# awslabs/palace

Hardware: AMD Instinct MI355X
Metric: curl-curl Mult DOF/s + PCG iters/s, p=3 H(curl) 10M DOF @1/2/4/8 GPU (higher is better)
Workload: dtype f64

## Files before the change

palace_amd/csrc/pa_internal.hpp:

```cpp
#pragma once

#include <hip/hip_runtime.h>

#include <cstdint>
#include <cstdio>
#include <memory>
#include <stdexcept>
#include <string>
#include <vector>

#include "../../include/palace_amd.h"
#include "pa_devbuf.hpp"
#include "pa_stream_host.hpp"

struct pa_op;
typedef struct pa_op pa_op_fwd;

struct pa_csr {
  bool symmetric = true;
  int32_t nrows = 0;
  int32_t ncols = 0;
  int64_t nnz = 0;
  pa::DevBuf<int32_t> d_rowptr, d_col;
  pa::DevBuf<double> d_val;
// ... 70 lines not shown
  DevBuf<double> d_geom;
  Ref<QData> metric;
  DevBuf<int32_t> d_attr_e;
  std::vector<int32_t> h_attr;
  std::vector<int32_t> eorder;
  std::vector<double> w1;
  DevBuf<double> d_xnodes, d_gtab;
  std::vector<double> wq;
  int refcount = 1;
  virtual ~Geom() = default;
};

struct CoeffDev {
  const int32_t *attr_mat = nullptr;
  const double *mat = nullptr;
  int nattr = 0;
};

struct CoeffHost {
  std::vector<int32_t> attr_mat;
  std::vector<double> mat;
  int dim = 3;
  size_t slots = 0;
  DevBuf<int32_t> d_attr_mat;
  DevBuf<double> d_mat;
  DevBuf<double> d_mat_t;
  bool symmetric() const { return !d_mat_t; }
  CoeffDev dev() const;
};

struct TransposeScope {
  TransposeScope(bool on);
  ~TransposeScope();
  static bool active();

private:
  bool prev_;
};

__host__ __device__ inline int nd_qd_cstride(int q1d) { return q1d == 5 ? 126 : q1d * q1d * q1d; }
__host__ __device__ inline int nd_qd_offset(int q1d, int c, int q) {
  if (q1d == 4) return ((c * 2 + (q >> 5)) * 16 + (q & 15)) * 2 + ((q >> 4) & 1);
  if (q1d == 5) {
    const int qz = q / 25, t = q - 25 * qz;
    return c * 126 + (qz < 4 ? (qz >> 1) * 50 + 2 * t + (qz & 1) : 100 + t);
  }
  return c * q1d * q1d * q1d + q;
}

enum StreamForm { kStreamPlain = 0, kStreamMasked = 1, kStreamAll = 2 };
inline StreamForm stream_form(bool masked) { return masked ? kStreamMasked : kStreamPlain; }

struct StreamTables {
  DevBuf<uint32_t> d_flags;
  DevBuf<uint32_t> d_rchunk;
  DevBuf<int32_t> d_rhdr;
  DevBuf<int32_t> d_rpos;
  int n_rows = 0, n_runs = 0;
  bool ready() const { return d_rhdr != nullptr; }
};

struct SubOp {
  Ref<Geom> geom;
  Ref<QData> qd;
  int fe_type = 0, p = 0, q1d = 0, P = 0, Q = 0, ne = 0, lsize = 0;
  int qf = 0;
  uint32_t trial_ops = 0, test_ops = 0;
  DevBuf<int32_t> d_lidx;
  DevBuf<int32_t> d_sidx;
  DevBuf<int32_t> d_sidx_bc;
  DevBuf<uint16_t> d_perm;
  DevBuf<uint16_t> d_perm_x;
  DevBuf<int32_t> d_shared;
  DevBuf<int32_t> d_shared_bc;
  std::vector<int32_t> h_shared;
  int n_shared = 0;
  std::vector<uint16_t> h_perm;
  std::vector<int32_t> h_sidx;
  DevBuf<double> d_ye;
  DevBuf<double> d_ye2;
  DevBuf<int32_t> d_tptr;
  DevBuf<int32_t> d_tent;
  DevBuf<uint32_t> d_idxc;
  bool stream_default = true;
  std::vector<uint32_t> h_perm_s;
  DevBuf<uint32_t> d_slots;
  int n_slot_patterns = 0;
  DevBuf<double> d_coef_s;
  std::vector<char> h_ess_flag;
  StreamTables stream[3];
  std::vector<double> Bc, Gc, Bo;
  DevBuf<double> d_tab;
  bool iso = false;
  std::vector<uint8_t> ctx_blob;
  CoeffHost c0, c1;
};

struct DenseSub {
  Ref<Geom> geom;
  int fe_type = 0, P = 0, Q = 0, Qpad = 0, nch = 0, ne = 0, nb = 0, lsize = 0, KP = 0, PT = 0;
  int qf = 0, mode = 0;
  bool contra = false;
  bool ye_rows = false;
  uint32_t trial_ops = 0, test_ops = 0;
  DevBuf<int32_t> d_idx;
  DevBuf<int32_t> d_idx_bc;
  DevBuf<uint8_t> d_ess_flag;
  DevBuf<uint16_t> d_co;
  DevBuf<uint32_t> d_co2;
  DevBuf<int32_t> d_rows;
  int n_rows = 0;
  std::vector<int32_t> h_idx;
  std::vector<int32_t> h_off;
  DevBuf<double> d_Tf, d_Tt;
  DevBuf<double> d_L;
  DevBuf<double> d_qdata;
  std::vector<uint16_t> h_co;
  double chk_interp = 0.0, chk_deriv = 0.0;
  DevBuf<double> d_ye2;
  DevBuf<uint8_t> d_affine;
  DevBuf<double> d_wrel;
  int n_affine = 0;
  DevBuf<int32_t> d_blist[2];
  int n_blist[2] = {0, 0};
  int L_rows = 0, ncq = 0, num_cu = 0;
  DevBuf<double> d_interp, d_deriv;
  DevBuf<int32_t> d_off;
  DevBuf<int8_t> d_cor;
  DevBuf<uint8_t> d_ori;
  DevBuf<double> d_ye;
  DevBuf<int32_t> d_tptr, d_tent;
  std::vector<uint8_t> ctx_blob;
  CoeffHost c0, c1;
};

struct MixedSide {
  int fe_type = 0, P = 0, lsize = 0, nc = 3;
  std::vector<int32_t> h_off;
  DevBuf<int32_t> d_sidx;
  DevBuf<int8_t> d_cor;
  DevBuf<double> d_tabF, d_tabT;
  DevBuf<int32_t> d_tptr, d_tent;
};
struct MixedSub {
  Ref<Geom> geom;
  int ne = 0, Q = 0, qf = 0, kind = 0;
  bool error = false;
  MixedSide s1, s2;
  CoeffHost c0, c1;
  DevBuf<double> d_ye;
  mutable DevBuf<double> d_ye_t;
  std::unique_ptr<SubOp> hex1, hex2;
  DevBuf<int32_t> d_eorder;
};

void parse_coeff(const void *blob, size_t bytes, int dim, CoeffHost &out, size_t slot_offset);

void launch_geom(const pa_mesh_desc &mesh, Geom &g, hipStream_t s);
void launch_nd_hex_apply(const SubOp &so, const double *x, double *y, double *ye, bool masked, hipStream_t s,
                         bool accumulate = true, int ess_policy = -1, const double *x1 = nullptr, double *y1 = nullptr,
                         double *ye1 = nullptr);
bool nd_hex_supports_two_rhs(const SubOp &so);
void launch_et_gather2(const SubOp &so, double *y0, double *y1, bool accumulate, hipStream_t s, const double *x0,
                       const double *x1, int ess_policy);
bool nd_hex_fuses_essential(const SubOp &so);
void finalize_exclusive(pa_op_fwd *op);
// ... 141 lines not shown
```

palace_amd/csrc/pa_nd_hex_stream.hip:

```cpp
#include <algorithm>
#include <map>

#include "pa_nd_hex_core.hpp"
#include "pa_stream_launch.hpp"

namespace pa {

typedef double d2v __attribute__((ext_vector_type(2)));

__host__ __device__ constexpr int stream_lds_elem(const int raw) { return (raw + 15) / 32 * 32 + 16; }

template <int P1>
struct NDStreamArgs {
  int ne, nbatch, chunk;
  const uint32_t *idxc;
  const uint32_t *flagw;
  const uint32_t *slots;
  const double *qdata;
  const double *qaff;
  const double *qcol;
  double wq2[2];
  double wqi2[2];
  const double *coef;
  const double *xn, *gtab;
  const double *x;
  double *y, *ye;
  const double *x1, *coef1;
  double *y1, *ye1;
  const double *qdata1;
  int qm[2], qc[2], qn[2];
  int nsplit;
  const double *xg0, *xg1;
  const unsigned long long *xg_sel;
  double *yg;
  NDTab<P1, 4> tab;
};

template <int P1, bool USE_U, bool USE_C, bool METRIC, int MINW, int GPOS, bool CPLX = false, bool SPLIT = false, int GEOMN = 0,
          bool COMPACT = false>
__global__ __launch_bounds__(64 * kWavesPerBlock, MINW) void nd_hex_stream_kernel(const NDStreamArgs<P1> a) {
  static_assert(!COMPACT || (!CPLX && !GEOMN), "the compact-only form: real kernels on packed or metric data");
  static_assert(!CPLX || (USE_U && USE_C), "the complex form is built on the curl-curl + mass kernels");
  static_assert(!(CPLX && SPLIT), "no split-vector form of the complex kernel");
  static_assert(!GEOMN || (!USE_U && USE_C && !METRIC && !CPLX), "geometry from the nodes: the curl-curl kernel");
  constexpr int Q1 = 4;
  constexpr bool AFF = (!CPLX || METRIC) && !GEOMN;
  constexpr bool EARLY_IDX = P1 < 3;
  using L = typename std::conditional<P1 == 3 && !CPLX && USE_C && !USE_U, NDLayoutInPlaceSwz3, NDLayout<P1, Q1>>::type;
  constexpr int NC = P1 + 1, PP = 3 * P1 * NC * NC, NPL = (PP + 15) / 16, NPK = (NPL + 3) / 4;
  constexpr int NG = METRIC ? (USE_U ? 7 : 6) : 6 * ((USE_U ? 1 : 0) + (USE_C ? 1 : 0));
  static_assert(PP <= 256, "8-bit slots");
  using streamhost::kIdxPattern;
  using streamhost::kIdxStart0;
  using streamhost::kIdxWords;
  constexpr int LDS_SIDE = (PP + 1) / 2 + (NPK + 1) * 8;
  constexpr int LDS_XN = GEOMN ? 82 : 0;
  constexpr int LDS_ELEM = stream_lds_elem(L::ELEM_PAD + LDS_SIDE + 12 + LDS_XN);
  extern __shared__ __attribute__((aligned(16))) double smem[];
  const int lane = threadIdx.x & 63;
  const int wave = __builtin_amdgcn_readfirstlane(threadIdx.x >> 6);
  const int xcd = blockIdx.x & 7;
  const int base = xcd * a.chunk, bend = min(base + a.chunk, a.nbatch);
  const int stride = (int)(gridDim.x >> 3) * kWavesPerBlock;
  int b = base + (int)(blockIdx.x >> 3) * kWavesPerBlock + wave;
  if (b >= bend) return;
  const double *xsel = (CPLX && ((lane >> 4) & 1)) ? a.x1 : a.x;
  const double *xgh = nullptr;
  if (SPLIT) xgh = ((a.xg_sel ? *a.xg_sel : 0ull) & 1ull) ? a.xg1 : a.xg0;
  auto load_idx = [&](const int bb, const int sub, const int t, int (&s)[NPL + 2], unsigned (&p)[NPK + 1]) {
    const int e = CPLX ? bb * 2 + (sub >> 1) : bb * 4 + sub;
    const uint32_t *ic = a.idxc + (size_t)e * kIdxWords;
#pragma unroll
    for (int r = 0; r < NPL; r++) s[r] = (int)__builtin_nontemporal_load(&ic[r]);
    s[NPL] = (int)__builtin_nontemporal_load(&ic[kIdxStart0 + t]);
    s[NPL + 1] = (int)__builtin_nontemporal_load(&ic[kIdxStart0 + 16 + (t & 3)]);
    p[NPK] = __builtin_nontemporal_load(&a.flagw[(size_t)e * 16 + t]);
    p[0] = __builtin_nontemporal_load(&ic[kIdxPattern]);
  };
  auto gather = [&](int (&s)[NPL + 2], unsigned (&p)[NPK + 1], double (&xv)[NPL], int *stab, const int t) {
    stab[t] = s[NPL];
    if (t < 4) stab[16 + t] = s[NPL + 1];
    wave_sync();
    const unsigned fw = p[NPK];
    {
      const uint32_t *sl = a.slots + (size_t)p[0] * (NPK * 16) + t;
#pragma unroll
      for (int k = 0; k < NPK; k++) p[k] = sl[16 * k];
    }
#pragma unroll
    for (int r = 0; r < NPL; r++) {
      const unsigned w = (unsigned)s[r], low = (w & 0xffffu) & ((2u << t) - 1u);
      const int rid = (int)((w >> 16) & 31u) + __popc(low) - 1;
      const int pos = low ? 16 * r + 31 - __clz((int)low) : (int)((w >> 21) & 255u);
      int dof = stab[rid] + (t + 16 * r - pos);
      if (!(16 * r + 15 < PP) && t + 16 * r >= PP) dof = 0;
      xv[r] = SPLIT ? (dof < a.nsplit ? xsel : xgh)[dof] : xsel[dof];
      const int word = dof | ((fw >> (2 * r + 1)) & 1u ? kExclBit : 0) | ((fw >> (18 + r)) & 1u ? kEssBit : 0);
      s[r] = (fw >> (2 * r)) & 1u ? -1 - word : word;
    }
  };
  auto settle = [&](unsigned (&p)[NPK + 1]) { asm volatile("" : "+v"(p[NPK])); };
  int sA[NPL + 2];
  unsigned pA[NPK + 1];
  double xv[NPL];
  load_idx(b, lane >> 4, lane & 15, sA, pA);
  gather(sA, pA, xv,
         reinterpret_cast<int *>(smem + (size_t)(wave * 4 + (lane >> 4)) * LDS_ELEM + L::ELEM_PAD + LDS_SIDE), lane & 15);
#pragma unroll
  for (int r = 0; r < NPL; r++) asm volatile("" : "+v"(xv[r]));
  settle(pA);

  d2v gq[(GEOMN || COMPACT) ? 1 : 2 * NG];
  double gr[COMPACT ? NG : 1];
  double xl[GEOMN ? 6 : 1];
  auto load_xn = [&](const int ee, const int t) {
    const double *xp = a.xn + (size_t)ee * 81;
#pragma unroll
    for (int r = 0; r < (GEOMN ? 6 : 1); r++) xl[r] = (t + 16 * r < 81) ? __builtin_nontemporal_load(&xp[t + 16 * r]) : 0.0;
  };
  auto load_q = [&](const int ee, const int t, const int kind) {
    if (GEOMN) return load_xn(ee, t);
    if (COMPACT) {
      constexpr int NS = METRIC ? 7 : NG;
      const int rs = kind == 2 ? 4 : 16;
      const double *g = kind == 2 ? a.qaff + ((size_t)ee * (4 * NS) + (t & 1)) : a.qcol + ((size_t)ee * (NS * 16) + t);
#pragma unroll
      for (int c = 0; c < NG; c++) gr[c] = __builtin_nontemporal_load(&g[rs * c]);
      return;
    }
    if (AFF && !(CPLX && !METRIC)) {
      constexpr int NS = METRIC ? 7 : NG;
      const int rs = kind == 2 ? 1 : (kind == 1 ? 4 : 16);
      const d2v *g = kind == 2   ? reinterpret_cast<const d2v *>(a.qaff) + (size_t)ee * (2 * NS)
                     : kind == 1 ? reinterpret_cast<const d2v *>(a.qcol) + ((size_t)ee * (NS * 8) + (t >> 1))
                                 : reinterpret_cast<const d2v *>(a.qdata) + ((size_t)ee * (2 * NS * 16) + t);
#pragma unroll
      for (int k = 0; k < 2 * NG; k++) gq[k] = __builtin_nontemporal_load(&g[rs * k]);
      return;
    }
    if (CPLX && !METRIC) {
      const int grp = (lane >> 4) & 1;
      const int mo = a.qm[grp], co = a.qc[grp];
      const d2v *g = reinterpret_cast<const d2v *>(grp ? a.qdata1 : a.qdata) + ((size_t)ee * (2 * a.qn[grp] * 16) + t);
      const d2v zero = {0.0, 0.0};
#pragma unroll
      for (int k = 0; k < 12; k++) {
        gq[k] = mo >= 0 ? __builtin_nontemporal_load(&g[16 * (2 * mo + k)]) : zero;
        gq[12 + k] = co >= 0 ? __builtin_nontemporal_load(&g[16 * (2 * co + k)]) : zero;
      }
      return;
    }
    const d2v *g = reinterpret_cast<const d2v *>(a.qdata) + ((size_t)ee * (2 * (METRIC ? 7 : NG) * 16) + t);
#pragma unroll
    for (int k = 0; k < (GEOMN ? 1 : 2 * NG); k++) gq[k] = __builtin_nontemporal_load(&g[16 * k]);
  };
  for (;;) {
    int lo;
    asm volatile("v_mbcnt_lo_u32_b32 %0, -1, 0\n\tv_mbcnt_hi_u32_b32 %0, -1, %0" : "=v"(lo));
    const int sub = lo >> 4, t = lo & 15, ta = t & 3, tb = t >> 2;
    double *sm = smem + (size_t)(wave * 4 + sub) * LDS_ELEM;
    int *side = reinterpret_cast<int *>(sm + L::ELEM_PAD);
    int *stab = side + 2 * LDS_SIDE;
    constexpr int lx = 0;
    const int e = CPLX ? b * 2 + (sub >> 1) : b * 4 + sub;

    const int kind = AFF ? __builtin_amdgcn_readfirstlane((int)(pA[NPK] >> 30)) : 0;
    const int aff = kind >> 1, col = kind & 1;
    load_q(e, t, kind);
    d2v ce = {0.0, 0.0}, ci = {0.0, 0.0};
    if (METRIC || GEOMN) ce = reinterpret_cast<const d2v *>(a.coef)[e];
    if (CPLX && METRIC) ci = reinterpret_cast<const d2v *>(a.coef1)[e];

#pragma unroll
    for (int r = 0; r < NPL; r++) {
      if (16 * r + 15 < PP || t + 16 * r < PP) {
        const int sv = sA[r], df = sv >= 0 ? sv : -1 - sv;
        const double v = (df & kEssBit) ? 0.0 : xv[r];
        sm[(pA[r >> 2] >> (8 * (r & 3))) & 255u] = sv >= 0 ? v : -v;
        side[t + 16 * r] = sv;
      }
    }
#pragma unroll
    for (int k = 0; k <= NPK; k++) side[2 * ((PP + 1) / 2) + 16 * k + t] = (int)pA[k];
    wave_sync();
    double uin[3][NC];
#pragma unroll
    for (int C = 0; C < 3; C++) {
      const int ni = (C == 0) ? P1 : NC, nj = (C == 1) ? P1 : NC, nk = (C == 2) ? P1 : NC;
      const bool act = ta < nj && tb < nk;
#pragma unroll
      for (int i = 0; i < NC; i++) uin[C][i] = (act && i < ni) ? sm[C * P1 * NC * NC + i + ni * (ta + nj * tb)] : 0.0;
    }
    wave_sync();

    const int kn = b + stride;
    const bool more = kn < bend;
    const int bn = more ? kn : b;
    int sB[NPL + 2];
    unsigned pB[NPK + 1];
    if (EARLY_IDX) {
      load_idx(bn, sub, t, sB, pB);
      __builtin_amdgcn_sched_barrier(0);
    }
    double U[3][Q1], CU[3][Q1];
#pragma unroll
    for (int c = 0; c < 3; c++)
#pragma unroll
      for (int q = 0; q < Q1; q++) U[c][q] = 0.0, CU[c][q] = 0.0;
    nd_fwd_comp<0, P1, Q1, USE_U, USE_C, L>(a, e, true, true, ta, tb, lx, sm, uin[0], U, CU);
    nd_fwd_comp<1, P1, Q1, USE_U, USE_C, L>(a, e, true, true, ta, tb, lx, sm, uin[1], U, CU);
    nd_fwd_comp<2, P1, Q1, USE_U, USE_C, L>(a, e, true, true, ta, tb, lx, sm, uin[2], U, CU);

    if (!EARLY_IDX) {
      __builtin_amdgcn_sched_barrier(0);
      load_idx(bn, sub, t, sB, pB);
      __builtin_amdgcn_sched_barrier(0);
    }

    constexpr bool PARK = GEOMN == 2;
    double Pz[GEOMN ? 3 : 1][3][PARK ? 1 : 3];
    double Pl = 0.0;
    double cw = 0.0;
    double *xs = sm + L::ELEM_PAD + LDS_SIDE + 12;
    auto park = [&](const int q) -> double * { return (q < 12 ? sm + 16 * q : xs + 16 * (q - 12)) + t; };
    if (GEOMN) {
#pragma unroll
      for (int r = 0; r < 6; r++)
        if (t + 16 * r < 81) xs[t + 16 * r] = xl[r];
      wave_sync();
      const double *gt = a.gtab;
      double bx[3], gx[3], by[3], gy[3];
#pragma unroll
      for (int i = 0; i < 3; i++) bx[i] = gt[ta * 3 + i], gx[i] = gt[12 + ta * 3 + i], by[i] = gt[tb * 3 + i], gy[i] = gt[12 + tb * 3 + i];
      cw = ce[1] * gt[24 + ta] * gt[24 + tb];
#pragma unroll
      for (int k = 0; k < 3; k++) {
        double acc[3][3];
#pragma unroll
        for (int c = 0; c < 3; c++) acc[c][0] = 0.0, acc[c][1] = 0.0, acc[c][2] = 0.0;
#pragma unroll
        for (int j = 0; j < 3; j++) {
#pragma unroll
          for (int i = 0; i < 3; i++) {
            const double w0 = gx[i] * by[j], w1 = bx[i] * gy[j], w2 = bx[i] * by[j];
            const double *X = xs + 3 * (i + 3 * (j + 3 * k));
#pragma unroll
            for (int c = 0; c < 3; c++) {
              const double xc = X[c];
              acc[c][0] += xc * w0, acc[c][1] += xc * w1, acc[c][2] += xc * w2;
            }
          }
        }
        if (PARK && k == 2) wave_sync();
#pragma unroll
        for (int c = 0; c < 3; c++) {
          Pz[k][c][0] = acc[c][0];
          if (!PARK) {
            Pz[k][c][PARK ? 0 : 1] = acc[c][1], Pz[k][c][PARK ? 0 : 2] = acc[c][2];
          } else {
            *park(6 * k + 2 * c) = acc[c][1];
            if (k == 2 && c == 2) Pl = acc[c][2]; else *park(6 * k + 2 * c + 1) = acc[c][2];
          }
        }
        if (PARK) __builtin_amdgcn_sched_barrier(0);
      }
    }
// ... 83 lines not shown
        }
        if (USE_U) {
          const double cm = H[6] * cmass;
          const double m[6] = {cm * (H[3] * H[5] - H[4] * H[4]), cm * (H[2] * H[4] - H[1] * H[5]), cm * (H[1] * H[4] - H[2] * H[3]),
                               cm * (H[0] * H[5] - H[2] * H[2]), cm * (H[1] * H[2] - H[0] * H[4]), cm * (H[0] * H[3] - H[1] * H[1])};
          sym_mv(m, U[0][qz], U[1][qz], U[2][qz], U[0][qz], U[1][qz], U[2][qz]);
        }
        if (USE_C) {
          const double m[6] = {ccurl * H[0], ccurl * H[1], ccurl * H[2], ccurl * H[3], ccurl * H[4], ccurl * H[5]};
          sym_mv(m, CU[0][qz], CU[1][qz], CU[2][qz], CU[0][qz], CU[1][qz], CU[2][qz]);
        }
        if (AFF) {
#pragma unroll
          for (int c = 0; c < 3; c++) {
            if (USE_U) U[c][qz] *= wab;
            if (USE_C) CU[c][qz] *= wab;
          }
        }
        __builtin_amdgcn_sched_barrier(0);
      } else if (CPLX) {
        const bool im = sub & 1;
#pragma unroll
        for (int f = 0; f < 2; f++) {
          double(&W)[3][Q1] = f ? CU : U;
          double ur[3], ui[3], ar[3], ai[3];
#pragma unroll
          for (int c = 0; c < 3; c++) {
            const double pv = __shfl_xor(W[c][qz], 16, 64);
            ur[c] = im ? pv : W[c][qz], ui[c] = im ? W[c][qz] : pv;
          }
          sym_mv(&H[6 * f], ur[0], ur[1], ur[2], ar[0], ar[1], ar[2]);
          sym_mv(&H[6 * f], ui[0], ui[1], ui[2], ai[0], ai[1], ai[2]);
#pragma unroll
          for (int c = 0; c < 3; c++) {
            const double got = __shfl_xor(ai[c], 16, 64);
            W[c][qz] = im ? ar[c] + got : ar[c] - got;
          }
        }
        __builtin_amdgcn_sched_barrier(0);
      } else {
        if (USE_U) sym_mv(&H[0], U[0][qz], U[1][qz], U[2][qz], U[0][qz], U[1][qz], U[2][qz]);
        if (USE_C) sym_mv(&H[USE_U ? 6 : 0], CU[0][qz], CU[1][qz], CU[2][qz], CU[0][qz], CU[1][qz], CU[2][qz]);
        if (AFF) {
#pragma unroll
          for (int c = 0; c < 3; c++) {
            if (USE_U) U[c][qz] *= wab;
            if (USE_C) CU[c][qz] *= wab;
          }
        }
      }
    }

    if (GEOMN == 2) wave_sync();

    double xB[NPL];
    nd_bwd_comp<0, P1, Q1, USE_U, USE_C, L>(a, e, true, true, ta, tb, lx, sm, uin[0], U, CU);
    if (GPOS == 1) {
      __builtin_amdgcn_sched_barrier(0);
      gather(sB, pB, xB, stab, t);
      settle(pB);
      __builtin_amdgcn_sched_barrier(0);
    }
    nd_bwd_comp<1, P1, Q1, USE_U, USE_C, L>(a, e, true, true, ta, tb, lx, sm, uin[1], U, CU);
    if (GPOS == 2) {
      __builtin_amdgcn_sched_barrier(0);
      gather(sB, pB, xB, stab, t);
      settle(pB);
      __builtin_amdgcn_sched_barrier(0);
    }
    nd_bwd_comp<2, P1, Q1, USE_U, USE_C, L>(a, e, true, true, ta, tb, lx, sm, uin[2], U, CU);

#pragma unroll
    for (int C = 0; C < 3; C++) {
      const int ni = (C == 0) ? P1 : NC, nj = (C == 1) ? P1 : NC, nk = (C == 2) ? P1 : NC;
      const bool act = ta < nj && tb < nk;
#pragma unroll
      for (int i = 0; i < NC; i++)
        if (act && i < ni) sm[C * P1 * NC * NC + i + ni * (ta + nj * tb)] = uin[C][i];
    }
    wave_sync();
#pragma unroll
    for (int r = 0; r < NPL; r++) {
      const int m = (16 * r + 15 < PP) ? t + 16 * r : min(t + 16 * r, PP - 1), mt = m & 15, mr = m >> 4;
      const unsigned fl = (unsigned)side[2 * ((PP + 1) / 2) + 16 * NPK + mt] >> (2 * mr);
      const double v = sm[((unsigned)side[2 * ((PP + 1) / 2) + 16 * (mr >> 2) + mt] >> (8 * (mr & 3))) & 255u];
      const int sv = side[m], df = sv >= 0 ? sv : -1 - sv, d = df & (kExclBit - 1);
      double *yd = (CPLX && (sub & 1)) ? a.y1 : a.y;
      if (SPLIT) yd = d < a.nsplit ? a.y : a.yg;
      double *dst = (fl & 2u) ? yd + d : ((CPLX && (sub & 1)) ? a.ye1 : a.ye) + ((size_t)e * PP + m);
      *dst = (fl & 1u) ? -v : v;
    }
    wave_sync();
    if (!more) break;
    b = bn;
#pragma unroll
    for (int r = 0; r < NPL; r++) sA[r] = sB[r], xv[r] = xB[r];
#pragma unroll
    for (int k = 0; k <= NPK; k++) pA[k] = pB[k];
  }
}

using streamhost::RunHdr;
using streamhost::RunChunk;

constexpr int kGatherILP = 4;
struct GatherPart2 {
  const double *ye1, *x1;
  double *y1;
};
template <bool STEP, bool DUAL = false>
__global__ __launch_bounds__(256) void et_run_gather_kernel_t(const int n, const RunChunk *__restrict__ chunk,
                                                              const RunHdr *__restrict__ hdr, const int32_t *__restrict__ rpos,
                                                              const double *__restrict__ ye, double *__restrict__ y,
                                                              const int accumulate, const double *__restrict__ x,
                                                              const int ess_policy, const int nsplit, double *__restrict__ yg,
                                                              const GatherStep st, const GatherPart2 p2) {
  const int k0 = blockIdx.x * (256 * kGatherILP) + threadIdx.x;
  const int lane = threadIdx.x & 63;
  RunHdr h[kGatherILP];
  int pe[kGatherILP], d[kGatherILP], j[kGatherILP], run[kGatherILP];
  bool live[kGatherILP], fix[kGatherILP];
  double s[kGatherILP], yold[kGatherILP];
#pragma unroll
  for (int u = 0; u < kGatherILP; u++) {
    const int k = k0 + 256 * u;
    live[u] = k < n;
    const RunChunk c = chunk[live[u] ? (k >> 6) : 0];
    const unsigned long long low = (c.starts & ~1ull) & ((2ull << lane) - 1ull);
    const int nc = __popcll(low);
    run[u] = (int)(c.first >> 4) + nc;
    j[u] = nc ? lane - (63 - __clzll((long long)low)) : (int)(c.first & 15u) + lane;
  }
#pragma unroll
  for (int u = 0; u < kGatherILP; u++) {
    h[u] = hdr[live[u] ? run[u] : 0];
    pe[u] = hdr[live[u] ? run[u] + 1 : 0].ptr;
    fix[u] = (h[u].dof0 >> 31) && ess_policy >= 0;
  }
#pragma unroll
  for (int u = 0; u < kGatherILP; u++) {
    d[u] = (int)(h[u].dof0 & streamhost::kRunDofMask) + j[u];
    s[u] = 0.0;
    yold[u] = 0.0;
    if (live[u] && fix[u]) {
      if (ess_policy) s[u] = x[d[u]];
      pe[u] = h[u].ptr;
    } else if (!STEP && live[u] && accumulate) {
      yold[u] = y[d[u]];
    }
  }
  double se[STEP ? kGatherILP : 1], sdi[STEP ? kGatherILP : 1], sr0[STEP ? kGatherILP : 1], sep[STEP ? kGatherILP : 1],
      so[STEP ? kGatherILP : 1];
  if (STEP) {
#pragma unroll
    for (int u = 0; u < kGatherILP; u++) {
      const int dd = (live[u] && d[u] < nsplit) ? d[u] : 0;
      sr0[u] = st.r0[dd];
      sdi[u] = st.dinv ? st.dinv[dd] : 0.0;
      se[u] = st.mode == 1 ? x[dd] : 0.0;
      sep[u] = (st.mode == 1 && st.ep) ? st.ep[dd] : 0.0;
      so[u] = (st.mode == 1 && st.add) ? st.out[dd] : 0.0;
    }
  }
  int pos[kGatherILP][4];
#pragma unroll
  for (int u = 0; u < kGatherILP; u++)
#pragma unroll
    for (int q = 0; q < 4; q++) pos[u][q] = (live[u] && h[u].ptr + q < pe[u]) ? rpos[h[u].ptr + q] : -1;
  double v[kGatherILP][4];
// ... 173 lines not shown
    for (int e = 0; e < ne; e++) qd.n_aff_elems += flag[e] & 1;
    for (int b = 0; b < nep / 4; b++)
      if (flag[4 * b] & flag[4 * b + 1] & flag[4 * b + 2] & flag[4 * b + 3] & 1) qd.batch_aff[b] = 1, qd.n_aff_batch_elems += real_elems(b);
  }
  if (col_enabled) {
    qd.batch_col.assign((size_t)nep / 4, 0);
    for (int e = 0; e < ne; e++) qd.n_col_elems += (flag[e] >> 1) & 1;
    for (int b = 0; b < nep / 4; b++)
      if ((flag[4 * b] & flag[4 * b + 1] & flag[4 * b + 2] & flag[4 * b + 3] & 2) && !qd.batch_aff[b])
        qd.batch_col[b] = 1, qd.n_col_batch_elems += real_elems(b);
    if (qd.n_col_batch_elems == 0)
      qd.batch_col.clear();
    else
      qd.d_col = std::move(d_col);
  }
  qd.all_compact = nep > 0;
  for (int b = 0; b < nep / 4; b++) qd.all_compact = qd.all_compact && (qd.batch_aff[b] || (!qd.batch_col.empty() && qd.batch_col[b]));
  if (qd.n_aff_batch_elems == 0)
    qd.batch_aff.clear();
  else
    qd.d_aff = std::move(d_aff);
}

static streamhost::FlagLayout flag_layout(const SubOp &so) {
  return streamhost::FlagLayout{wide_form(so) ? streamhost::FlagLayout::kFlagWide : streamhost::FlagLayout::kFlagRow, so.P};
}

static DevBuf<uint32_t> upload_flags(const SubOp &so, const std::vector<uint32_t> &pp) {
  if (so.fe_type != PA_FE_HCURL || wide_form(so)) return dev_upload(pp.data(), pp.size());
  const std::vector<uint32_t> fw = streamhost::split_flag_rows(flag_layout(so), pp);
  return dev_upload(fw.data(), fw.size());
}

static void upload_runs(StreamTables &t, const SubOp &so, const std::vector<int32_t> &rows, const char *ess) {
  std::vector<uint32_t> code;
  std::vector<RunHdr> hdr;
  std::vector<int32_t> rpos;
  streamhost::build_runs(so.ne, so.P, so.lsize, so.h_sidx.data(), rows, code, hdr, rpos, ess);
  const std::vector<RunChunk> ch = streamhost::run_chunks(code);
  t.d_rchunk = dev_upload(reinterpret_cast<const uint32_t *>(ch.data()), 4 * ch.size());
  t.d_rhdr = dev_upload(reinterpret_cast<const int32_t *>(hdr.data()), 2 * hdr.size());
  t.d_rpos = dev_upload(rpos.data(), rpos.size());
  t.n_rows = (int)rows.size(), t.n_runs = (int)hdr.size() - 1;
}

void build_stream(SubOp &so) {
  if (so.d_idxc || !(nd_hex_stream_ok(so) || h1_hex_stream_capable(so))) return;
  const int P = so.P, ne = so.ne;
  const bool lane16_curl = so.fe_type == PA_FE_HCURL && !wide_form(so);
  const streamhost::FlagLayout fl = flag_layout(so);
  std::vector<uint32_t> ic, pp;
  if (wide_form(so)) {
    if (!streamhost::pack_index_wide(ne, P, so.lsize, so.h_sidx.data(), so.h_perm.data(), ic, pp)) return;
  } else if (!streamhost::pack_index(ne, P, so.lsize, so.h_sidx.data(), so.h_perm.data(), ic, pp,
                                     so.fe_type == PA_FE_H1 ? streamhost::kIdxStart0H1 : streamhost::kIdxStart0))
    return;
  if (lane16_curl) {
    stream_affine_setup(so);
    for (size_t b = 0; b < so.qd->batch_aff.size(); b++)
      if (so.qd->batch_aff[b])
        for (size_t e = 4 * b; e < 4 * b + 4; e++) streamhost::set_element_bit(fl, pp, e, streamhost::kAffBit);
    for (size_t b = 0; b < so.qd->batch_col.size(); b++)
      if (so.qd->batch_col[b])
        for (size_t e = 4 * b; e < 4 * b + 4; e++) streamhost::set_element_bit(fl, pp, e, streamhost::kColBit);
    const int nep = fl.padded(ne), sw = fl.elem_words() - 16;
    std::vector<uint32_t> slots;
    std::map<std::vector<uint32_t>, uint32_t> dict;
    std::vector<uint32_t> key((size_t)sw);
    for (int e = 0; e < nep; e++) {
      const uint32_t *row = &pp[(size_t)e * fl.elem_words()];
      key.assign(row, row + sw);
      auto it = dict.find(key);
      if (it == dict.end()) {
        it = dict.emplace(key, (uint32_t)dict.size()).first;
        slots.insert(slots.end(), key.begin(), key.end());
      }
      ic[(size_t)e * streamhost::kIdxWords + streamhost::kIdxPattern] = it->second;
    }
    so.n_slot_patterns = (int)dict.size();
    so.d_slots = dev_upload(slots.data(), slots.size());
  }
  so.h_perm_s = pp;
  so.d_idxc = dev_upload(ic.data(), ic.size());
  if (so.qd->metric || (so.iso && so.qf == PA_QF_HDIV_33 && so.geom->d_xnodes)) stream_element_coefficients(so);
  StreamTables &t = so.stream[kStreamPlain];
  t.d_flags = upload_flags(so, pp);
  upload_runs(t, so, so.h_shared, nullptr);
}

void stream_set_essential(SubOp &so, const std::vector<char> &flag) {
  if (!so.d_idxc) return;
  so.h_ess_flag = flag;
  so.stream[kStreamAll] = StreamTables{};
  std::vector<uint32_t> pb(so.h_perm_s);
  streamhost::mark_essential(flag_layout(so), pb, so.ne, so.h_sidx.data(), flag.data(), true);
  StreamTables &t = so.stream[kStreamMasked];
  t = StreamTables{};
  t.d_flags = upload_flags(so, pb);
  upload_runs(t, so, streamhost::gather_rows(so.ne, so.P, so.lsize, so.h_sidx.data(), flag.data(), false), flag.data());
}

template <int P1, bool U, bool C, bool METRIC, int MINW, int GPOS, bool CPLX = false, bool SPLIT = false, int GEOMN = 0,
          bool COMPACT = false>
static void launch_gpos(const SubOp &so, NDStreamArgs<P1> &a, hipStream_t s) {
  using L = typename std::conditional<P1 == 3 && !CPLX && C && !U, NDLayoutInPlaceSwz3, NDLayout<P1, 4>>::type;
  for (int i = 0; i < HalfTab<P1, 4>::LEN; i++) a.tab.Bo[i] = so.Bo[i];
  for (int i = 0; i < HalfTab<P1 + 1, 4>::LEN; i++) a.tab.Bc[i] = so.Bc[i], a.tab.Gc[i] = so.Gc[i];
  constexpr int PP = 3 * P1 * (P1 + 1) * (P1 + 1);
  constexpr int NPK = ((PP + 15) / 16 + 3) / 4;
  const size_t lds = sizeof(double) * (size_t)(kWavesPerBlock * 4) *
                     stream_lds_elem(L::ELEM_PAD + (PP + 1) / 2 + (NPK + 1) * 8 + 12 + (GEOMN ? 82 : 0));
  static const int wg_env = stream_env_int("PALACE_AMD_STREAM_WG");
  static const int per_cu_query =
      std::min({stream_occupancy(nd_hex_stream_kernel<P1, U, C, METRIC, MINW, GPOS, CPLX, SPLIT, GEOMN, COMPACT>, 64 * kWavesPerBlock, lds, 8),
                MINW * 4 / kWavesPerBlock, (int)(160 * 1024 / lds), 8});
  if (CPLX) a.nbatch = (so.ne + 1) / 2;
  else a.nbatch = (so.ne + 3) / 4;
  if (a.nbatch == 0) return;
  a.chunk = (a.nbatch + 7) / 8;
  const int wgx = stream_wgx(wg_env > 0 ? wg_env : per_cu_query, a.chunk, kWavesPerBlock, false);
  hipLaunchKernelGGL((nd_hex_stream_kernel<P1, U, C, METRIC, MINW, GPOS, CPLX, SPLIT, GEOMN, COMPACT>), dim3(8 * wgx), dim3(64 * kWavesPerBlock),
                     lds, s, a);
  PA_HIP(hipGetLastError());
}

template <int P1, bool U, bool C, bool METRIC, int MINW, bool COMPACT = false>
static void launch_variant(const SubOp &so, NDStreamArgs<P1> &a, hipStream_t s) {
  constexpr int GPOS = U ? 2 : 1;
  constexpr bool RAISE = COMPACT && C && ((U && P1 < 3) || (!U && METRIC && P1 == 3));
  constexpr int W = RAISE ? 3 : MINW;
  if (a.nsplit >= 0)
    return launch_gpos<P1, U, C, METRIC, W, GPOS, false, true, 0, COMPACT>(so, a, s);
  launch_gpos<P1, U, C, METRIC, W, GPOS, false, false, 0, COMPACT>(so, a, s);
}

bool nd_hex_stream_compact(const SubOp &so) {
  if (!so.qd || !so.qd->all_compact || so.fe_type != PA_FE_HCURL || so.q1d != 4 || !so.d_idxc) return false;
  const char *e = getenv("PALACE_AMD_STREAM_COMPACT");
  return !(e && atoi(e) == 0);
}
template <int P1, bool U, bool C, bool METRIC, int MINW>
static void launch_form(const SubOp &so, NDStreamArgs<P1> &a, hipStream_t s) {
  if (nd_hex_stream_compact(so)) return launch_variant<P1, U, C, METRIC, MINW, true>(so, a, s);
  launch_variant<P1, U, C, METRIC, MINW>(so, a, s);
}

template <int P1>
static void launch_p(const SubOp &so, const double *x, double *y, StreamForm form, hipStream_t s, const SplitIO *split) {
  NDStreamArgs<P1> a{};
  stream_set_split(a, split, so.lsize);
  a.ne = so.ne, a.nbatch = 0;
  a.idxc = so.d_idxc;
  a.flagw = so.stream[form].d_flags;
  a.slots = so.d_slots;
  a.qdata = so.qd->d;
  a.qaff = so.qd->d_aff, a.qcol = so.qd->d_col, a.wq2[0] = so.qd->wq2[0], a.wq2[1] = so.qd->wq2[1];
  if (so.qd->d_col) a.wqi2[0] = 1.0 / so.qd->wq2[0], a.wqi2[1] = 1.0 / so.qd->wq2[1];
  a.coef = so.d_coef_s;
  a.xn = nullptr, a.gtab = nullptr;
  a.x = x, a.y = y, a.ye = so.d_ye;
  const bool m = so.qd->metric;
  switch (so.qf) {
    case PA_QF_HDIV_33: {
      const char *ge = getenv("PALACE_AMD_STREAM_GEOM");
      const bool geomn = ge && std::string(ge) == "nodes";
      if (!m && geomn && P1 == 3 && so.iso && so.geom->d_xnodes && so.d_coef_s && !split) {
        a.xn = so.geom->d_xnodes, a.gtab = so.geom->d_gtab;
        const char *ve = getenv("PALACE_AMD_GEOMN_VARIANT");
        if (ve && std::string(ve) == "w2g2") launch_gpos<P1, false, true, false, 2, 2, false, false, (P1 == 3 ? 1 : 0)>(so, a, s);
        else if (ve && std::string(ve) == "park3g1") launch_gpos<P1, false, true, false, 3, 1, false, false, (P1 == 3 ? 2 : 0)>(so, a, s);
        else if (ve && std::string(ve) == "park3g2") launch_gpos<P1, false, true, false, 3, 2, false, false, (P1 == 3 ? 2 : 0)>(so, a, s);
        else launch_gpos<P1, false, true, false, 2, 1, false, false, (P1 == 3 ? 1 : 0)>(so, a, s);
        break;
      }
      if (m) launch_form<P1, false, true, true, (P1 == 3 ? 2 : 3)>(so, a, s); else launch_form<P1, false, true, false, 3>(so, a, s);
    } break;
    case PA_QF_HCURL_33:
      if (m) launch_form<P1, true, false, true, 3>(so, a, s); else launch_form<P1, true, false, false, 3>(so, a, s);
      break;
    case PA_QF_HDIVMASS_33:
      if (m) launch_form<P1, true, true, true, 2>(so, a, s);
      else launch_form<P1, true, true, false, 2>(so, a, s);
      break;
    default: throw Error("QFunction not available for H(curl) hexahedra");
  }
}

void launch_nd_hex_stream_all(const SubOp &so, const double *x, hipStream_t s, const SplitIO *split) {
  PA_REQUIRE(so.stream[kStreamAll].ready(), "stream_build_all has not been called");
  launch_nd_hex_stream(so, x, so.d_ye, kStreamAll, s, split);
}

bool nd_hex_stream_split_ok(const SubOp &so) {
  return so.fe_type == PA_FE_HCURL && so.d_idxc &&
         (so.q1d == 4 || (wide_form(so) && nd_hex_stream5_ok(so)) || (three_point_form(so) && nd_hex_stream3_ok(so)));
}

void launch_nd_hex_stream(const SubOp &so, const double *x, double *y, StreamForm form, hipStream_t s, const SplitIO *split) {
  if (so.fe_type == PA_FE_H1) return launch_h1_hex_stream(so, x, y, form, s, split);
  if (wide_form(so)) return launch_nd_hex_stream5(so, x, y, form, s, split);
  if (three_point_form(so)) return launch_nd_hex_stream3(so, x, y, form, s, split);
  switch (so.p) {
    case 1: launch_p<1>(so, x, y, form, s, split); break;
    case 2: launch_p<2>(so, x, y, form, s, split); break;
    case 3: launch_p<3>(so, x, y, form, s, split); break;
    default: throw Error("no streaming H(curl) hex kernel for this order");
  }
}

bool nd_hex_stream_complex_ok(const SubOp &sr, const SubOp &si) {
  static const bool enabled = !(getenv("PALACE_AMD_COMPLEX_FUSED") && atoi(getenv("PALACE_AMD_COMPLEX_FUSED")) == 0);
  auto qf_ok = [](const SubOp &so) {
    return so.fe_type == PA_FE_HCURL && (so.qf == PA_QF_HDIV_33 || so.qf == PA_QF_HCURL_33 || so.qf == PA_QF_HDIVMASS_33);
  };
  if (!enabled || !qf_ok(sr) || !qf_ok(si)) return false;
  if (sr.geom != si.geom || sr.ne != si.ne || sr.p != si.p || sr.P != si.P || sr.q1d != si.q1d) return false;
  auto iso_ok = [](const SubOp &so) {
    return so.iso && ((so.q1d == 4 && so.p <= 3) || (so.q1d == 5 && so.p <= 4 && nd_hex_stream5_ok(so))) && !so.geom->h_attr.empty();
  };
  const bool metric = iso_ok(sr) && iso_ok(si) && sr.d_idxc && sr.d_coef_s && sr.qd && sr.qd->metric;
  auto packed_ok = [](const SubOp &so) {
    return ((so.q1d == 4 && so.p <= 3) || (so.q1d == 5 && so.p <= 4 && nd_hex_stream5_ok(so))) && so.qd && !so.qd->metric &&
           so.qd->ncomp == (so.qf == PA_QF_HDIVMASS_33 ? 12 : 6);
  };
  const bool packed = packed_ok(sr) && packed_ok(si) && sr.d_idxc;
  if (!metric && !packed) return false;
  return sr.h_sidx == si.h_sidx;
}

template <int P1>
static void launch_complex_p(const SubOp &sr, const SubOp &si, const double *xr, const double *xi, double *yr, double *yi,
                             double *ye_i, bool masked, hipStream_t s) {
  NDStreamArgs<P1> a{};
  a.ne = sr.ne, a.nbatch = 0;
  a.idxc = sr.d_idxc;
// ... 84 lines not shown
```

palace_amd/csrc/pa_stream_host.hpp:

```cpp
#pragma once

#include <cstdint>
#include <stdexcept>
#include <vector>

namespace pa {

constexpr int kEssBit = 1 << 30;
constexpr int kExclBit = 1 << 29;

namespace streamhost {

struct RunHdr {
  uint32_t dof0;
  int32_t ptr;
};
constexpr uint32_t kRunDofMask = (1u << 27) - 1u;
inline int run_dof0(const RunHdr &h) { return (int)(h.dof0 & kRunDofMask); }
inline int run_len(const RunHdr &h) { return (int)((h.dof0 >> 27) & 15u) + 1; }
inline bool run_ess(const RunHdr &h) { return (h.dof0 >> 31) != 0; }

inline int dof_of(int32_t s) { return s >= 0 ? s : -1 - s; }

constexpr int kIdxWords = 32, kIdxStart0 = 12, kIdxMaxRuns = kIdxWords - kIdxStart0, kIdxStart0H1 = 4;
constexpr int kIdxPattern = 11;
constexpr uint32_t kAffBit = 1u << 31;
constexpr uint32_t kColBit = 1u << 30;

inline int index_dof(const uint32_t *ic, int m, int start0 = kIdxStart0) {
  const int r = m >> 4, t = m & 15;
  const uint32_t w = ic[r], low = (w & 0xffffu) & ((2u << t) - 1u);
  int bits = 0, top = -1;
  for (int j = 0; j < 16; j++)
    if (low >> j & 1u) bits++, top = j;
  const int rid = (int)((w >> 16) & 31u) + bits - 1;
  if (rid < 0 || rid >= kIdxWords - start0) throw std::runtime_error("index decode: entry without a run");
  const int pos = low ? 16 * r + top : (int)((w >> 21) & 255u);
  return (int)ic[start0 + rid] + (m - pos);
}

inline bool pack_index(int ne, int P, int lsize, const int32_t *sidx, const uint16_t *perm, std::vector<uint32_t> &ic,
                       std::vector<uint32_t> &pp, int start0 = kIdxStart0) {
  if (P > 256) throw std::runtime_error("element too large for 8-bit slots");
  if (lsize >= kExclBit) throw std::runtime_error("too many local dofs for the streaming index encoding");
  const int nep = (ne + 3) & ~3, npl = (P + 15) / 16, npk = (npl + 3) / 4;
  if (npl > 9 || npl > start0) throw std::runtime_error("element too large for the flag word / slice words");
  const int max_runs = kIdxWords - start0;
  const size_t nnz = (size_t)ne * P;
  std::vector<int32_t> count((size_t)lsize, 0);
  for (size_t k = 0; k < nnz; k++) count[dof_of(sidx[k])]++;
  ic.assign((size_t)nep * kIdxWords, 0u);
  pp.assign((size_t)nep * (npk + 1) * 16, 0u);
  for (int e = 0; e < nep; e++) {
    uint32_t *ice = &ic[(size_t)e * kIdxWords];
    if (e >= ne) {
      ice[0] = 1u;
      for (int r = 1; r < npl; r++) ice[r] = 1u << 16;
      continue;
    }
    int nruns = 0, lastpos = 0, prev = -2;
    for (int m = 0; m < P; m++) {
      const size_t k = (size_t)e * P + m;
      const int32_t s = sidx[k];
      const int d = dof_of(s);
      const int t = m & 15, r = m >> 4;
      if (t == 0) ice[r] |= (uint32_t)nruns << 16 | (uint32_t)lastpos << 21;
      if (d != prev + 1) {
        if (nruns == max_runs) return false;
        ice[start0 + nruns++] = (uint32_t)d;
        ice[r] |= 1u << t;
        lastpos = m;
      }
      prev = d;
      const bool excl = count[d] == 1;
      uint32_t *row = &pp[(size_t)e * (npk + 1) * 16];
      row[(r >> 2) * 16 + t] |= (uint32_t)(perm[k] & 0xff) << (8 * (r & 3));
      row[npk * 16 + t] |= ((s < 0 ? 1u : 0u) | (excl ? 2u : 0u)) << (2 * r);
    }
  }
  return true;
}

constexpr int kWideWords = 48, kWideStart0 = 20, kWideMaxRuns = 24, kWideMaxSlices = 10;
constexpr uint32_t kWideSlotMask = 511u, kWideFlip = 1u << 9, kWideExcl = 1u << 10, kWideEss = 1u << 11;

inline int index_dof_wide(const uint32_t *ic, int m) {
  const int r = m >> 5, t = m & 31;
  const uint32_t w = ic[2 * r], info = ic[2 * r + 1], low = w & ((2u << t) - 1u);
  int bits = 0, top = -1;
  for (int j = 0; j < 32; j++)
    if (low >> j & 1u) bits++, top = j;
  const int rid = (int)(info & 255u) + bits - 1;
  if (rid < 0 || rid >= kWideMaxRuns) throw std::runtime_error("wide index decode: entry without a run");
  const int pos = low ? 32 * r + top : (int)((info >> 8) & 511u);
  return (int)ic[kWideStart0 + rid] + (m - pos);
}

inline bool pack_index_wide(int ne, int P, int lsize, const int32_t *sidx, const uint16_t *perm, std::vector<uint32_t> &ic,
                            std::vector<uint32_t> &pp) {
  if (P > 32 * kWideMaxSlices) throw std::runtime_error("element too large for the wide streaming index");
  if (lsize >= kExclBit) throw std::runtime_error("too many local dofs for the streaming index encoding");
  const int nep = (ne + 1) & ~1, npl = (P + 31) / 32, npk = (npl + 1) / 2;
  const size_t nnz = (size_t)ne * P;
  std::vector<int32_t> count((size_t)lsize, 0);
  for (size_t k = 0; k < nnz; k++) count[dof_of(sidx[k])]++;
  ic.assign((size_t)nep * kWideWords, 0u);
  pp.assign((size_t)nep * npk * 32, 0u);
  for (int e = 0; e < nep; e++) {
    uint32_t *ice = &ic[(size_t)e * kWideWords];
    uint32_t *row = &pp[(size_t)e * npk * 32];
    if (e >= ne) {
      ice[0] = 1u;
      for (int r = 1; r < npl; r++) ice[2 * r + 1] = 1u;
      for (int m = 0; m < P; m++) row[(m >> 6) * 32 + (m & 31)] |= ((uint32_t)m | kWideEss) << (16 * ((m >> 5) & 1));
      continue;
    }
    int nruns = 0, lastpos = 0, prev = -2;
    for (int m = 0; m < P; m++) {
      const size_t k = (size_t)e * P + m;
      const int32_t s = sidx[k];
      const int d = dof_of(s);
      const int t = m & 31, r = m >> 5;
      if (t == 0) ice[2 * r + 1] = (uint32_t)nruns | (uint32_t)lastpos << 8;
      if (d != prev + 1) {
        if (nruns == kWideMaxRuns) return false;
        ice[kWideStart0 + nruns++] = (uint32_t)d;
        ice[2 * r] |= 1u << t;
        lastpos = m;
      }
      prev = d;
      const uint32_t h = (uint32_t)(perm[k] & kWideSlotMask) | (s < 0 ? kWideFlip : 0u) | (count[d] == 1 ? kWideExcl : 0u);
      row[(r >> 1) * 32 + t] |= h << (16 * (r & 1));
    }
  }
  return true;
}

struct FlagLayout {
  enum Kind { kFlagRow, kFlagSplit, kFlagWide } kind;
  int P;
  int lanes() const { return kind == kFlagWide ? 32 : 16; }
  int slices() const { return (P + lanes() - 1) / lanes(); }
  int padded(int ne) const { return kind == kFlagWide ? (ne + 1) & ~1 : (ne + 3) & ~3; }
  int elem_words() const {
    return kind == kFlagWide ? (slices() + 1) / 2 * 32 : (kind == kFlagSplit ? 16 : ((slices() + 3) / 4 + 1) * 16);
  }
  size_t word(size_t e, int m) const {
    const int t = m & (lanes() - 1), r = m / lanes();
    if (kind == kFlagWide) return e * elem_words() + (r >> 1) * 32 + t;
    return (e + 1) * elem_words() - 16 + t;
  }
  int half(int m) const { return 16 * ((m >> 5) & 1); }
  uint32_t flipped(int m) const { return kind == kFlagWide ? kWideFlip << half(m) : 1u << (2 * (m >> 4)); }
  uint32_t only_copy(int m) const { return kind == kFlagWide ? kWideExcl << half(m) : 2u << (2 * (m >> 4)); }
  uint32_t essential(int m) const { return kind == kFlagWide ? kWideEss << half(m) : 1u << (18 + (m >> 4)); }
};

inline void clear_only_copy(const FlagLayout &fl, std::vector<uint32_t> &w) {
  const size_t nep = w.size() / fl.elem_words();
  for (size_t e = 0; e < nep; e++)
    for (int m = 0; m < fl.slices() * fl.lanes(); m++) w[fl.word(e, m)] &= ~fl.only_copy(m);
}
inline void mark_essential(const FlagLayout &fl, std::vector<uint32_t> &w, size_t e, int m, bool off_direct) {
  uint32_t &f = w[fl.word(e, m)];
// ... 142 lines not shown
```

Before: 70.95 billion.

## Use plain per-element DOF index array in compact curl-curl stream kernel

For the compact kernel variant, stores a plain per-element signed DOF index table (one int per local DOF, padded to 16) instead of decoding the run-length compressed index words. The gather skips the run decode and LDS staging of the run table. The scatter reads flags and slot words from registers, using wave shuffles for the padded tail, instead of from LDS side arrays. This cuts LDS footprint and decode ALU work, which may raise occupancy, but it reads several times more index bytes per element from global memory.

```diff
diff --git a/palace_amd/csrc/pa_internal.hpp b/palace_amd/csrc/pa_internal.hpp
--- a/palace_amd/csrc/pa_internal.hpp
+++ b/palace_amd/csrc/pa_internal.hpp
@@ -176,6 +176,7 @@
   DevBuf<int32_t> d_tptr;
   DevBuf<int32_t> d_tent;
   DevBuf<uint32_t> d_idxc;
+  DevBuf<int32_t> d_idxp;
   bool stream_default = true;
   std::vector<uint32_t> h_perm_s;
   DevBuf<uint32_t> d_slots;
diff --git a/palace_amd/csrc/pa_nd_hex_stream.hip b/palace_amd/csrc/pa_nd_hex_stream.hip
--- a/palace_amd/csrc/pa_nd_hex_stream.hip
+++ b/palace_amd/csrc/pa_nd_hex_stream.hip
@@ -34,6 +34,7 @@
   const unsigned long long *xg_sel;
   double *yg;
   NDTab<P1, 4> tab;
+  const int32_t *idxp;
 };
 
 template <int P1, bool USE_U, bool USE_C, bool METRIC, int MINW, int GPOS, bool CPLX = false, bool SPLIT = false, int GEOMN = 0,
@@ -53,9 +54,9 @@
   using streamhost::kIdxPattern;
   using streamhost::kIdxStart0;
   using streamhost::kIdxWords;
-  constexpr int LDS_SIDE = (PP + 1) / 2 + (NPK + 1) * 8;
+  constexpr int LDS_SIDE = COMPACT ? 0 : (PP + 1) / 2 + (NPK + 1) * 8;
   constexpr int LDS_XN = GEOMN ? 82 : 0;
-  constexpr int LDS_ELEM = stream_lds_elem(L::ELEM_PAD + LDS_SIDE + 12 + LDS_XN);
+  constexpr int LDS_ELEM = stream_lds_elem(L::ELEM_PAD + LDS_SIDE + (COMPACT ? 0 : 12) + LDS_XN);
   extern __shared__ __attribute__((aligned(16))) double smem[];
   const int lane = threadIdx.x & 63;
   const int wave = __builtin_amdgcn_readfirstlane(threadIdx.x >> 6);
@@ -70,6 +71,14 @@
   auto load_idx = [&](const int bb, const int sub, const int t, int (&s)[NPL + 2], unsigned (&p)[NPK + 1]) {
     const int e = CPLX ? bb * 2 + (sub >> 1) : bb * 4 + sub;
     const uint32_t *ic = a.idxc + (size_t)e * kIdxWords;
+    if (COMPACT) {
+      const int32_t *ip = a.idxp + ((size_t)e * (NPL * 16) + t);
+#pragma unroll
+      for (int r = 0; r < NPL; r++) s[r] = __builtin_nontemporal_load(&ip[16 * r]);
+      p[NPK] = __builtin_nontemporal_load(&a.flagw[(size_t)e * 16 + t]);
+      p[0] = __builtin_nontemporal_load(&ic[kIdxPattern]);
+      return;
+    }
 #pragma unroll
     for (int r = 0; r < NPL; r++) s[r] = (int)__builtin_nontemporal_load(&ic[r]);
     s[NPL] = (int)__builtin_nontemporal_load(&ic[kIdxStart0 + t]);
@@ -78,6 +87,18 @@
     p[0] = __builtin_nontemporal_load(&ic[kIdxPattern]);
   };
   auto gather = [&](int (&s)[NPL + 2], unsigned (&p)[NPK + 1], double (&xv)[NPL], int *stab, const int t) {
+    if (COMPACT) {
+      if (GPOS == 1 && bend < 0) return;
+      const uint32_t *sl = a.slots + (size_t)p[0] * (NPK * 16) + t;
+#pragma unroll
+      for (int k = 0; k < NPK; k++) p[k] = sl[16 * k];
+#pragma unroll
+      for (int r = 0; r < NPL; r++) {
+        const int dof = s[r] >= 0 ? s[r] : -1 - s[r];
+        xv[r] = SPLIT ? (dof < a.nsplit ? xsel : xgh)[dof] : xsel[dof];
+      }
+      return;
+    }
     stab[t] = s[NPL];
     if (t < 4) stab[16 + t] = s[NPL + 1];
     wave_sync();
@@ -175,13 +196,15 @@
     for (int r = 0; r < NPL; r++) {
       if (16 * r + 15 < PP || t + 16 * r < PP) {
         const int sv = sA[r], df = sv >= 0 ? sv : -1 - sv;
-        const double v = (df & kEssBit) ? 0.0 : xv[r];
+        const double v = (COMPACT ? (pA[NPK] >> (18 + r)) & 1u : df & kEssBit) ? 0.0 : xv[r];
         sm[(pA[r >> 2] >> (8 * (r & 3))) & 255u] = sv >= 0 ? v : -v;
-        side[t + 16 * r] = sv;
-      }
-    }
-#pragma unroll
-    for (int k = 0; k <= NPK; k++) side[2 * ((PP + 1) / 2) + 16 * k + t] = (int)pA[k];
+        if (!COMPACT) side[t + 16 * r] = sv;
+      }
+    }
+    if (!COMPACT) {
+#pragma unroll
+      for (int k = 0; k <= NPK; k++) side[2 * ((PP + 1) / 2) + 16 * k + t] = (int)pA[k];
+    }
     wave_sync();
     double uin[3][NC];
 #pragma unroll
@@ -431,9 +454,23 @@
 #pragma unroll
     for (int r = 0; r < NPL; r++) {
       const int m = (16 * r + 15 < PP) ? t + 16 * r : min(t + 16 * r, PP - 1), mt = m & 15, mr = m >> 4;
-      const unsigned fl = (unsigned)side[2 * ((PP + 1) / 2) + 16 * NPK + mt] >> (2 * mr);
-      const double v = sm[((unsigned)side[2 * ((PP + 1) / 2) + 16 * (mr >> 2) + mt] >> (8 * (mr & 3))) & 255u];
-      const int sv = side[m], df = sv >= 0 ? sv : -1 - sv, d = df & (kExclBit - 1);
+      unsigned wf, ws;
+      int sv;
+      if (COMPACT) {
+        wf = pA[NPK], ws = pA[r >> 2], sv = sA[r];
+        if (!(16 * r + 15 < PP)) {
+          const int src = (lo & ~15) | ((PP - 1) & 15);
+          const unsigned of = __shfl(wf, src, 64), os = __shfl(ws, src, 64);
+          const int ov = __shfl(sv, src, 64);
+          if (t + 16 * r >= PP) wf = of, ws = os, sv = ov;
+        }
+      } else {
+        wf = (unsigned)side[2 * ((PP + 1) / 2) + 16 * NPK + mt], ws = (unsigned)side[2 * ((PP + 1) / 2) + 16 * (mr >> 2) + mt];
+        sv = side[m];
+      }
+      const unsigned fl = wf >> (2 * mr);
+      const double v = sm[(ws >> (8 * (mr & 3))) & 255u];
+      const int df = sv >= 0 ? sv : -1 - sv, d = df & (kExclBit - 1);
       double *yd = (CPLX && (sub & 1)) ? a.y1 : a.y;
       if (SPLIT) yd = d < a.nsplit ? a.y : a.yg;
       double *dst = (fl & 2u) ? yd + d : ((CPLX && (sub & 1)) ? a.ye1 : a.ye) + ((size_t)e * PP + m);
@@ -773,6 +810,11 @@
   }
   so.h_perm_s = pp;
   so.d_idxc = dev_upload(ic.data(), ic.size());
+  if (so.q1d == 4 && lane16_curl && so.qd->all_compact) {
+    std::vector<int32_t> ip;
+    streamhost::pack_index_plain(ne, P, so.h_sidx.data(), ip);
+    so.d_idxp = dev_upload(ip.data(), ip.size());
+  }
   if (so.qd->metric || (so.iso && so.qf == PA_QF_HDIV_33 && so.geom->d_xnodes)) stream_element_coefficients(so);
   StreamTables &t = so.stream[kStreamPlain];
   t.d_flags = upload_flags(so, pp);
@@ -800,7 +842,7 @@
   constexpr int PP = 3 * P1 * (P1 + 1) * (P1 + 1);
   constexpr int NPK = ((PP + 15) / 16 + 3) / 4;
   const size_t lds = sizeof(double) * (size_t)(kWavesPerBlock * 4) *
-                     stream_lds_elem(L::ELEM_PAD + (PP + 1) / 2 + (NPK + 1) * 8 + 12 + (GEOMN ? 82 : 0));
+                     stream_lds_elem(L::ELEM_PAD + (COMPACT ? 0 : (PP + 1) / 2 + (NPK + 1) * 8 + 12) + (GEOMN ? 82 : 0));
   static const int wg_env = stream_env_int("PALACE_AMD_STREAM_WG");
   static const int per_cu_query =
       std::min({stream_occupancy(nd_hex_stream_kernel<P1, U, C, METRIC, MINW, GPOS, CPLX, SPLIT, GEOMN, COMPACT>, 64 * kWavesPerBlock, lds, 8),
@@ -826,7 +868,7 @@
 }
 
 bool nd_hex_stream_compact(const SubOp &so) {
-  if (!so.qd || !so.qd->all_compact || so.fe_type != PA_FE_HCURL || so.q1d != 4 || !so.d_idxc) return false;
+  if (!so.qd || !so.qd->all_compact || so.fe_type != PA_FE_HCURL || so.q1d != 4 || !so.d_idxc || !so.d_idxp) return false;
   const char *e = getenv("PALACE_AMD_STREAM_COMPACT");
   return !(e && atoi(e) == 0);
 }
@@ -841,7 +883,7 @@
   NDStreamArgs<P1> a{};
   stream_set_split(a, split, so.lsize);
   a.ne = so.ne, a.nbatch = 0;
-  a.idxc = so.d_idxc;
+  a.idxc = so.d_idxc, a.idxp = so.d_idxp;
   a.flagw = so.stream[form].d_flags;
   a.slots = so.d_slots;
   a.qdata = so.qd->d;
diff --git a/palace_amd/csrc/pa_stream_host.hpp b/palace_amd/csrc/pa_stream_host.hpp
--- a/palace_amd/csrc/pa_stream_host.hpp
+++ b/palace_amd/csrc/pa_stream_host.hpp
@@ -80,6 +80,14 @@
   }
   return true;
 }
+
+inline void pack_index_plain(int ne, int P, const int32_t *sidx, std::vector<int32_t> &ip) {
+  const int nep = (ne + 3) & ~3, row = (P + 15) / 16 * 16;
+  ip.assign((size_t)nep * row, 0);
+  for (int e = 0; e < ne; e++)
+    for (int m = 0; m < P; m++) ip[(size_t)e * row + m] = sidx[(size_t)e * P + m];
+}
+inline int index_dof_plain(const int32_t *ip, int m) { return dof_of(ip[m]); }
 
 constexpr int kWideWords = 48, kWideStart0 = 20, kWideMaxRuns = 24, kWideMaxSlices = 10;
 constexpr uint32_t kWideSlotMask = 511u, kWideFlip = 1u << 9, kWideExcl = 1u << 10, kWideEss = 1u << 11;
```

Result: faster. 72.79 billion, median of 6 (+2.6%).
